# HengyiWang/spann3r

Hardware: NVIDIA H100
Metric: frames/sec (512x384, 10-frame seq) enc->mem-attn->dec->DPT (higher is better)
Workload: dtype bf16x3 (split-bf16 operands, fp32 accumulate; tf32 attention)

## Files before the change

include/spann3r_b200.h:

```cpp
#ifndef SPANN3R_B200_H_
#define SPANN3R_B200_H_

#include <stddef.h>
#include <stdint.h>

#ifdef __cplusplus
extern "C" {
#endif

#define S3R_VERSION 100

enum { S3R_EPI_PLAIN = 0, S3R_EPI_PIXSHUF = 1, S3R_EPI_QKV = 2, S3R_EPI_HEADTAIL = 3 };
enum { S3R_ACT_NONE = 0, S3R_ACT_GELU = 1, S3R_ACT_RELU = 2 };

int s3r_version(void);
int s3r_abi_sizeof(int which );
const char* s3r_last_error(void);
int s3r_device_ok(void);


int s3r_split(const float* x, int64_t ldx, void* hi, void* lo, int64_t ldp, int col0, int64_t rows, int c, int relu,
              void* stream);

int s3r_layernorm(const float* x, int64_t ldx, const float* w, const float* b, int64_t wb_group_stride,
// ... 15 lines not shown
                   void* stream);
int s3r_col2im_3x3s2(const float* cols, int nb, int h, int w, int c, int ho, int wo, float* out, void* stream);

typedef struct s3r_gemm_desc {
  const void* a_hi; const void* a_lo;
  const void* b_hi; const void* b_lo;
  int groups, nb, h, w, kc, taps, n;
  int epi, act, plane_relu, force_bn;
  const float* bias;
  const float* res1; int64_t ldr1;
  const float* res2; int64_t ldr2;
  float* out_f32; int64_t ldo;
  void* out_hi; void* out_lo; int64_t ldp; int plane_col0;
  int ps_s, ps_cout;
  int q_c, q_role_base, q_ntok, q_ntok_pad, q_rope, q_nb;
  const int32_t* q_pos; const float* q_cs;
  float* q_out; float* k_out; float* vt_out; float q_scale;
  const float* ht_w; const float* ht_b; float* ht_pts; float* ht_conf;
  const float* ln_stats; int ln_np; float ln_eps; const float* ln_cs; int a_swap;
  float* stats_out;
  uint64_t* trace;
  int swap_col0; float* k2_out; float* vt2_out;
  int precision;
} s3r_gemm_desc;
int s3r_gemm(const s3r_gemm_desc* d, void* stream);
int s3r_gemm_tile_n(const s3r_gemm_desc* d);
int s3r_gemm_plan_bn(int64_t m_tiles, int n, int sms, int col_align, int force_bn);

int s3r_attention(const float* q, const float* k, const float* vt, int bh, int heads, int nq, int nk, int nk_pad,
                  void* o_hi, void* o_lo, float* o_f32, int64_t ldo, void* stream);

int s3r_conf_score(const float* conf, int64_t n, float* scratch256, float* out, void* stream);
int s3r_conf_score_batched(const float* conf, int batch, int64_t hw, float* scratch, float* out, void* stream);

int s3r_resample_h_u8(const uint8_t* src, int64_t row_stride, int rows, int out_cols, const int32_t* bounds,
                      const int32_t* kk, int ksize, int max_span, uint8_t* dst, void* stream);
int s3r_resample_v_u8_norm(const uint8_t* tmp, int cols, int out_rows, const int32_t* bounds, const int32_t* kk, int ksize,
                           float* dst, void* stream);

int s3r_focal_weiszfeld(const float* pts3d, int b, int h, int w, float ppx, float ppy, int iters, float lo, float hi,
                        float* scratch, float* focal, void* stream);

int s3r_focal_median(const float* pts3d, int b, int h, int w, float ppx, float ppy, float lo, float hi, int32_t* scratch,
                     float* focal, void* stream);

size_t s3r_pnp_workspace_bytes(int b, int n_samples);
int s3r_pnp_ransac(const float* pts3d, const float* img_pts, int b, int64_t n, int width, double fx, double fy, double cx,
                   double cy, float reproj_err, int n_samples, int refine_iters, uint64_t seed, void* workspace,
                   double* out, uint8_t* inlier_mask, void* stream);

// ... 177 lines not shown
```

spann3r_b200/_lib.py:

```python
from __future__ import annotations

import ctypes as C
import os

import torch

_HERE = os.path.dirname(os.path.abspath(__file__))
LIB_PATH = os.environ.get("S3R_LIB", os.path.join(_HERE, "libspann3r_b200.so"))

EPI_PLAIN, EPI_PIXSHUF, EPI_QKV, EPI_HEADTAIL = 0, 1, 2, 3
PRECISION_SPLIT, PRECISION_BF16 = 0, 1
ACT_NONE, ACT_GELU, ACT_RELU = 0, 1, 2

_vp, _i, _i64, _f = C.c_void_p, C.c_int, C.c_int64, C.c_float


class GemmDesc(C.Structure):
    _fields_ = [
        ("a_hi", _vp), ("a_lo", _vp), ("b_hi", _vp), ("b_lo", _vp),
        ("groups", _i), ("nb", _i), ("h", _i), ("w", _i), ("kc", _i), ("taps", _i), ("n", _i),
        ("epi", _i), ("act", _i), ("plane_relu", _i), ("force_bn", _i),
        ("bias", _vp),
        ("res1", _vp), ("ldr1", _i64),
        ("res2", _vp), ("ldr2", _i64),
        ("out_f32", _vp), ("ldo", _i64),
        ("out_hi", _vp), ("out_lo", _vp), ("ldp", _i64), ("plane_col0", _i),
        ("ps_s", _i), ("ps_cout", _i),
        ("q_c", _i), ("q_role_base", _i), ("q_ntok", _i), ("q_ntok_pad", _i), ("q_rope", _i), ("q_nb", _i),
        ("q_pos", _vp), ("q_cs", _vp),
        ("q_out", _vp), ("k_out", _vp), ("vt_out", _vp), ("q_scale", _f),
        ("ht_w", _vp), ("ht_b", _vp), ("ht_pts", _vp), ("ht_conf", _vp),
        ("ln_stats", _vp), ("ln_np", _i), ("ln_eps", _f), ("ln_cs", _vp), ("a_swap", _i),
        ("stats_out", _vp),
        ("trace", _vp),
        ("swap_col0", _i), ("k2_out", _vp), ("vt2_out", _vp),
        ("precision", _i),
    ]


class LossDesc(C.Structure):
    _fields_ = [
        ("frames", _i), ("batch", _i), ("height", _i), ("width", _i),
        ("norm_mode", _i), ("gt_scale", _i), ("fix_first", _i), ("shift_inv", _i), ("scale_inv", _i), ("conf_loss", _i),
        ("has_dist_clip", _i), ("alpha", _f), ("dist_clip", _f),
        ("pose0", _vp), ("gt_pts", C.POINTER(_vp)), ("valid", C.POINTER(_vp)), ("pred", C.POINTER(_vp)),
        ("conf", C.POINTER(_vp)),
    ]


LOSS_RES_HEADER, LOSS_RES_PER_B = 20, 6


class AttnTrainDesc(C.Structure):
    _fields_ = [
        ("batch", _i), ("heads", _i), ("nq", _i), ("nk", _i), ("dh", _i), ("scale", _f),
        ("q", _vp), ("k", _vp), ("v", _vp),
        ("q_stride", _i64 * 3), ("k_stride", _i64 * 3), ("v_stride", _i64 * 3),
    ]

_PROTOS = {
    "s3r_version": (_i, []),
    "s3r_abi_sizeof": (_i, [_i]),
    "s3r_last_error": (C.c_char_p, []),
    "s3r_device_ok": (_i, []),
    "s3r_split": (_i, [_vp, _i64, _vp, _vp, _i64, _i, _i64, _i, _i, _vp]),
    "s3r_layernorm": (_i, [_vp, _i64, _vp, _vp, _i64, _i64, _f, _i64, _i, _vp, _i64, _vp, _vp, _i64, _i, _i64, _vp]),
    "s3r_rope2d_inplace": (_i, [_vp, _vp, _i64, _i, _i, _i64, _i64, _f, _f, _vp]),
    "s3r_im2col_patch16": (_i, [_vp, _i64, _i64, _i64, _i64, _i, _i, _i, _vp, _vp, _vp]),
    "s3r_im2col_3x3s2": (_i, [_vp, _vp, _i, _i, _i, _i, _i, _i, _vp, _vp, _vp]),
    "s3r_upsample2x": (_i, [_vp, _i, _i, _i, _i, _vp, _vp, _vp, _vp]),
    "s3r_conv_wgrad_workspace_bytes": (C.c_size_t, [_i, _i, _i, _i, _i, _i]),
    "s3r_conv_wgrad": (_i, [_vp, _vp, _i64, _vp, _vp, _i64, _i, _i, _i, _i, _i, _i, _vp, C.c_size_t, _vp, _vp]),
    "s3r_col2im_3x3s2": (_i, [_vp, _i, _i, _i, _i, _i, _i, _vp, _vp]),
    "s3r_gemm": (_i, [C.POINTER(GemmDesc), _vp]),
    "s3r_gemm_tile_n": (_i, [C.POINTER(GemmDesc)]),
    "s3r_gemm_plan_bn": (_i, [_i64, _i, _i, _i, _i]),
    "s3r_attention": (_i, [_vp, _vp, _vp, _i, _i, _i, _i, _i, _vp, _vp, _vp, _i64, _vp]),
    "s3r_conf_score": (_i, [_vp, _i64, _vp, _vp, _vp]),
    "s3r_conf_score_batched": (_i, [_vp, _i, _i64, _vp, _vp, _vp]),
    "s3r_dropout_mask": (_i, [_vp, _i64, C.c_uint64, _f, _vp]),
    "s3r_set_option": (_i, [C.c_char_p, _i]),
    "s3r_focal_weiszfeld": (_i, [_vp, _i, _i, _i, _f, _f, _i, _f, _f, _vp, _vp, _vp]),
    "s3r_focal_median": (_i, [_vp, _i, _i, _i, _f, _f, _f, _f, _vp, _vp, _vp]),
    "s3r_pnp_workspace_bytes": (C.c_size_t, [_i, _i]),
    "s3r_pnp_ransac": (_i, [_vp, _vp, _i, _i64, _i, C.c_double, C.c_double, C.c_double, C.c_double, _f, _i, _i, C.c_uint64,
                            _vp, _vp, _vp, _vp]),
    "s3r_pcl_index_bytes": (C.c_size_t, [_i64]),
    "s3r_pcl_index_build": (_i, [_vp, _i, _i64, _vp, _vp, _vp]),
    "s3r_pcl_nearest": (_i, [_vp, _i64, _vp, _i, _i64, _vp, C.c_double, _vp, _vp, _vp]),
    "s3r_pcl_normals": (_i, [_vp, _i64, _i, _vp, _vp]),
    "s3r_pcl_icp_workspace_bytes": (C.c_size_t, []),
    "s3r_pcl_icp": (_i, [_vp, _i, _i64, _vp, _i64, C.c_double, _vp, _i, C.c_double, C.c_double, _vp, _vp, _vp]),
    "s3r_pcl_stats_workspace_bytes": (C.c_size_t, []),
    "s3r_pcl_stats": (_i, [_vp, _i64, C.c_double, _vp, _vp, _vp]),
    "s3r_pcl_abs_dot": (_i, [_vp, _vp, _vp, _i64, _vp, _vp]),
    "s3r_render_workspace_bytes": (C.c_size_t, [_i, _i]),
    "s3r_render_clear": (_i, [_vp, _i, _i, _vp]),
    "s3r_render_splat": (_i, [_vp, _vp, _i64, _i64, _vp, C.c_double, _i, _i, _vp, _vp]),
    "s3r_render_resolve": (_i, [_vp, _vp, _i, _i, _vp, _vp]),
# ... 225 lines not shown
```

spann3r_b200/csrc/capi.cu:

```cuda
#include "../../include/spann3r_b200.h"

#include <cstring>

#include "gemm.cuh"
#include "kernels.cuh"

using namespace s3r;

static inline cudaStream_t S(void* s) { return reinterpret_cast<cudaStream_t>(s); }
static inline __nv_bfloat16* B(void* p) { return reinterpret_cast<__nv_bfloat16*>(p); }
static inline const __nv_bfloat16* B(const void* p) { return reinterpret_cast<const __nv_bfloat16*>(p); }

extern "C" {

int s3r_version(void) { return S3R_VERSION; }
int s3r_abi_sizeof(int which) {
  switch (which) {
    case 0: return (int)sizeof(s3r_gemm_desc);
    case 1: return (int)sizeof(s3r_model_w);
    case 2: return (int)sizeof(s3r_bank);
    case 3: return (int)sizeof(s3r_loss_desc);
    case 4: return (int)sizeof(s3r_attn_train_desc);
  }
  return -1;
// ... 129 lines not shown
    }
    if (d->ln_np < 2 || d->ln_np > 32 || d->ln_np % 2 != 0) {
      set_error("s3r_gemm: folded LayerNorm needs an even ln_np in [2, 32] (kc %% 64 == 0, kc <= 1024), got ln_np=%d",
                d->ln_np);
      return -1;
    }
  }
  if (d->swap_col0 % 256 != 0) {
    set_error("s3r_gemm: swap_col0 must be a multiple of 256");
    return -1;
  }
  if (d->stats_out && d->epi != S3R_EPI_PLAIN) {
    set_error("s3r_gemm: stats_out needs EPI_PLAIN");
    return -1;
  }
  return 0;
}

static int fill_plan(const s3r_gemm_desc* d, GemmPlan* plan) {
  int r = check_desc(d);
  if (r) return r;
  const int force_bn = d->epi == S3R_EPI_HEADTAIL ? (d->force_bn == 128 ? 128 : 1128) : d->force_bn;
  r = gemm_plan_init(plan, B(d->a_hi), B(d->a_lo), B(d->b_hi), B(d->b_lo), d->groups, d->nb, d->h, d->w, d->kc,
                     d->taps, d->n, force_bn, 0, 0, 0, d->precision, d->a_swap ? d->swap_col0 : 0);
  if (r) return r;
  GemmArgs& a = plan->args;
  a.epi = d->epi; a.act = d->act; a.plane_relu = d->plane_relu;
  a.bias = d->bias;
  a.res1 = d->res1; a.ldr1 = (int)d->ldr1;
  a.res2 = d->res2; a.ldr2 = (int)d->ldr2;
  a.out_f32 = d->out_f32; a.ldo = (int)d->ldo;
  a.out_hi = B(d->out_hi); a.out_lo = B(d->out_lo); a.ldp = (int)d->ldp; a.plane_col0 = d->plane_col0;
  if (d->epi == S3R_EPI_PIXSHUF) {
    a.ps_s = d->ps_s; a.ps_cout = d->ps_cout;
    a.out_group_rows = (long long)d->nb * d->h * d->ps_s * d->w * d->ps_s;
  }
  if (d->epi == S3R_EPI_QKV) {
    a.q_C = d->q_c; a.q_role_base = d->q_role_base; a.q_ntok = d->q_ntok; a.q_ntok_pad = d->q_ntok_pad;
    a.q_rope = d->q_rope; a.q_nb = d->q_nb; a.q_pos = d->q_pos;
    a.q_cs = reinterpret_cast<const float2*>(d->q_cs);
    a.q_out = d->q_out; a.k_out = d->k_out; a.vt_out = d->vt_out; a.q_scale = d->q_scale;
    a.k2_out = d->k2_out; a.vt2_out = d->vt2_out;
  }
  if (d->epi == S3R_EPI_HEADTAIL) {
    a.ht_w = d->ht_w; a.ht_b = d->ht_b; a.ht_pts = d->ht_pts; a.ht_conf = d->ht_conf;
  }
  if (d->ln_stats) {
    a.ln_stats = reinterpret_cast<const float2*>(d->ln_stats); a.ln_np = d->ln_np; a.ln_eps = d->ln_eps; a.ln_cs = d->ln_cs;
  }
  a.a_swap = d->a_swap ? 1 : 0;
  a.swap_col0 = d->swap_col0;
  a.stats_out = reinterpret_cast<float2*>(d->stats_out);
  a.trace = reinterpret_cast<unsigned long long*>(d->trace);
  return 0;
}

int s3r_gemm(const s3r_gemm_desc* d, void* stream) {
  GemmPlan plan;
  int r = fill_plan(d, &plan);
  if (r) return r;
  return gemm_launch(plan, S(stream));
}

int s3r_gemm_tile_n(const s3r_gemm_desc* d) {
  GemmPlan plan;
  int r = fill_plan(d, &plan);
  if (r) return r;
  return plan.bn;
}

int s3r_gemm_plan_bn(int64_t m_tiles, int n, int sms, int col_align, int force_bn) {
  if (m_tiles < 1 || n < 1 || sms < 1 || col_align < 0) {
    set_error("s3r_gemm_plan_bn: m_tiles=%lld n=%d sms=%d col_align=%d (positive; col_align >= 0)", (long long)m_tiles,
              n, sms, col_align);
    return -1;
  }
  return gemm_choose_bn(m_tiles, n, sms, col_align, force_bn);
}

int s3r_resample_h_u8(const uint8_t* src, int64_t row_stride, int rows, int out_cols, const int32_t* bounds,
                      const int32_t* kk, int ksize, int max_span, uint8_t* dst, void* stream) {
  return launch_resample_h_u8(src, row_stride, rows, out_cols, bounds, kk, ksize, max_span, dst, S(stream));
}
int s3r_resample_v_u8_norm(const uint8_t* tmp, int cols, int out_rows, const int32_t* bounds, const int32_t* kk, int ksize,
                           float* dst, void* stream) {
  return launch_resample_v_u8_norm(tmp, cols, out_rows, bounds, kk, ksize, dst, S(stream));
}

int s3r_focal_weiszfeld(const float* pts3d, int b, int h, int w, float ppx, float ppy, int iters, float lo, float hi,
                        float* scratch, float* focal, void* stream) {
  return launch_focal_weiszfeld(pts3d, b, h, w, ppx, ppy, iters, lo, hi, scratch, focal, S(stream));
}

// ... 62 lines not shown
  return launch_loss_backward(d, workspace, workspace_bytes, upstream, grad_pred, grad_conf, S(stream));
}

size_t s3r_attn_train_workspace_bytes(const s3r_attn_train_desc* d) { return attn_train_workspace_bytes(d); }
int s3r_attn_train_forward(const s3r_attn_train_desc* d, float* o, float* lse, void* stream) {
  return launch_attn_train_forward(d, o, lse, S(stream));
}
int s3r_attn_train_backward(const s3r_attn_train_desc* d, const float* o, const float* lse, const float* d_o,
                            void* workspace, size_t workspace_bytes, float* dq, float* dk, float* dv, void* stream) {
  return launch_attn_train_backward(d, o, lse, d_o, workspace, workspace_bytes, dq, dk, dv, S(stream));
}

int s3r_conf_score(const float* conf, int64_t n, float* scratch256, float* out, void* stream) {
  return launch_conf_score(conf, n, scratch256, out, S(stream));
}
int s3r_conf_score_batched(const float* conf, int batch, int64_t hw, float* scratch, float* out, void* stream) {
  return launch_conf_score_batched(conf, batch, hw, scratch, out, S(stream));
}

int s3r_set_option(const char* name, int value) {
  s3r::Options& o = s3r::options();
  if (!name) { set_error("s3r_set_option: null name"); return -1; }
  if (!strcmp(name, "prefetch_b")) o.prefetch_b = value;
  else { set_error("s3r_set_option: unknown option '%s' (prefetch_b)", name); return -1; }
  return 0;
}

int s3r_dropout_mask(float* out, int64_t n, uint64_t seed, float p, void* stream) {
  if (!out && n > 0) {
    set_error("s3r_dropout_mask: null output");
    return -1;
  }
  return launch_dropout_mask(out, n, seed, p, S(stream));
}

int s3r_attention(const float* q, const float* k, const float* vt, int bh, int heads, int nq, int nk, int nk_pad,
                  void* o_hi, void* o_lo, float* o_f32, int64_t ldo, void* stream) {
  return launch_attention(q, k, vt, bh, heads, nq, nk, nk_pad, B(o_hi), B(o_lo), o_f32, ldo, S(stream));
}

}
```

spann3r_b200/csrc/common.cuh:

```cuda
#pragma once
#include <cuda.h>
#include <cuda_bf16.h>
#include <cuda_runtime.h>
#include <stdint.h>

#include <cstdlib>
#include <utility>

namespace s3r {

__device__ __forceinline__ uint32_t smem_u32(const void* p) {
  return static_cast<uint32_t>(__cvta_generic_to_shared(p));
}
__device__ __forceinline__ uint32_t lane_id() { return threadIdx.x & 31; }
__device__ __forceinline__ bool elect_one() {
  uint32_t pred = 0;
  asm volatile(
      "{\n\t.reg .pred P1;\n\t"
      "elect.sync _|P1, 0xffffffff;\n\t"
      "selp.u32 %0, 1, 0, P1;\n\t}\n"
      : "=r"(pred));
  return pred != 0;
}

// ... 84 lines not shown
      "l"(reinterpret_cast<uint64_t>(m)), "r"(smem_u32(bar)), "r"(c0), "r"(c1), "r"(c2), "r"(c3)
      : "memory");
}

__device__ __forceinline__ void mbar_arrive_expect_tx_u(uint32_t bar, uint32_t bytes) {
  asm volatile("mbarrier.arrive.expect_tx.shared::cta.b64 _, [%0], %1;" ::"r"(bar), "r"(bytes) : "memory");
}
__device__ __forceinline__ void tma_load_3d_u(uint32_t smem, const CUtensorMap* m, uint32_t bar, int c0, int c1, int c2) {
  asm volatile(
      "cp.async.bulk.tensor.3d.shared::cta.global.mbarrier::complete_tx::bytes [%0], [%1, {%3, %4, %5}], [%2];" ::
          "r"(smem),
      "l"(reinterpret_cast<uint64_t>(m)), "r"(bar), "r"(c0), "r"(c1), "r"(c2)
      : "memory");
}
__device__ __forceinline__ void tma_load_4d_u(uint32_t smem, const CUtensorMap* m, uint32_t bar, int c0, int c1, int c2,
                                              int c3) {
  asm volatile(
      "cp.async.bulk.tensor.4d.shared::cta.global.mbarrier::complete_tx::bytes [%0], [%1, {%3, %4, %5, %6}], "
      "[%2];" ::"r"(smem),
      "l"(reinterpret_cast<uint64_t>(m)), "r"(bar), "r"(c0), "r"(c1), "r"(c2), "r"(c3)
      : "memory");
}

__device__ __forceinline__ uint64_t wgmma_desc_sw128_kmajor(uint32_t smem_addr) {
  uint64_t d = 0;
  d |= (uint64_t)((smem_addr & 0x3FFFF) >> 4);
  d |= (uint64_t)1 << 16;
  d |= (uint64_t)64 << 32;
  d |= (uint64_t)1 << 62;
  return d;
}

__device__ __forceinline__ uint64_t wgmma_desc_sw64_kmajor(uint32_t smem_addr) {
  uint64_t d = 0;
  d |= (uint64_t)((smem_addr & 0x3FFFF) >> 4);
  d |= (uint64_t)1 << 16;
  d |= (uint64_t)32 << 32;
  d |= (uint64_t)2 << 62;
  return d;
}

__device__ __forceinline__ void pdl_launch_dependents() { asm volatile("griddepcontrol.launch_dependents;" ::: "memory"); }
__device__ __forceinline__ void pdl_wait() { asm volatile("griddepcontrol.wait;" ::: "memory"); }

__device__ __forceinline__ unsigned long long globaltimer_ns() {
  unsigned long long t;
  asm volatile("mov.u64 %0, %%globaltimer;" : "=l"(t));
  return t;
}

__device__ __forceinline__ void st_f4(float* p, float a, float b, float c, float d) {
  *reinterpret_cast<float4*>(p) = make_float4(a, b, c, d);
}

struct PerDeviceOnce {
  bool done[64] = {};
  bool& cur() {
    int d = 0;
    cudaGetDevice(&d);
    return done[d & 63];
  }
};

template <typename... KArgs, typename... Args>
inline cudaError_t launch_pdl(void (*kernel)(KArgs...), dim3 grid, dim3 block, size_t smem, cudaStream_t st, Args&&... args) {
  cudaLaunchConfig_t cfg = {};
  cfg.gridDim = grid;
  cfg.blockDim = block;
  cfg.dynamicSmemBytes = smem;
  cfg.stream = st;
  static const bool use_pdl = (getenv("S3R_NO_PDL") == nullptr);
  cudaLaunchAttribute attr[1];
  attr[0].id = cudaLaunchAttributeProgrammaticStreamSerialization;
  attr[0].val.programmaticStreamSerializationAllowed = 1;
  cfg.attrs = attr;
  cfg.numAttrs = use_pdl ? 1 : 0;
  return cudaLaunchKernelEx(&cfg, kernel, std::forward<Args>(args)...);
}

}
```

spann3r_b200/csrc/gemm.cu:

```cuda
#include "gemm.cuh"

#include <cmath>
#include <cstdarg>
#include <cstdio>
#include <cstring>

#include "common.cuh"
#include "gemm_epilogue.cuh"
#include "wgmma.cuh"

namespace s3r {

static constexpr int BM = 128;
static constexpr int BK = 32;
static constexpr CUtensorMapSwizzle kSwizzle = CU_TENSOR_MAP_SWIZZLE_64B;
static constexpr int kEpiWarps = 8;
static constexpr int kNumThreads = 128 + 32 * kEpiWarps;
static constexpr int kSmemMax = 227 * 1024;
static constexpr int kAccLD = 36;
static constexpr int kAccBytes = 2 * BM * kAccLD * 4;

template <int BN, int NP>
struct GemmCfg {
  static constexpr int PLANES = NP == 3 ? 2 : 1;
// ... 22 lines not shown

template <int BN, int EPI, int NP>
__global__ void __launch_bounds__(kNumThreads, 1) gemm_bf16x3_kernel(const __grid_constant__ GemmArgs args) {
  using Cfg = GemmCfg<BN, NP>;
  extern __shared__ uint8_t smem_raw[];
  uint8_t* smem = smem_raw + ((1024u - (smem_u32(smem_raw) & 1023u)) & 1023u);
  uint64_t* bars = reinterpret_cast<uint64_t*>(smem + Cfg::STAGES * Cfg::STAGE);
  uint64_t* full_bar = bars;
  uint64_t* empty_bar = bars + Cfg::STAGES;
  float* sacc = reinterpret_cast<float*>(smem + Cfg::STAGES * Cfg::STAGE + 256);
  float* colv = reinterpret_cast<float*>(reinterpret_cast<uint8_t*>(sacc) + kAccBytes);
  float4* hts = reinterpret_cast<float4*>(reinterpret_cast<uint8_t*>(colv) + Cfg::COLV);

  const int warp = threadIdx.x >> 5;
  const int lane = threadIdx.x & 31;
  const bool trace = blockIdx.x == 0 && args.trace != nullptr;
  if (trace && threadIdx.x == 0) args.trace[0] = globaltimer_ns();

  const int n_tiles = (args.N + BN - 1) / BN;
  const int m_tiles = args.tiles_w * args.tiles_h * args.NB;
  const int tiles_per_group = n_tiles * m_tiles;
  const int total_tiles = tiles_per_group * args.groups;
  const int num_kb = args.taps * args.kpt;

  if (warp == 0 && lane == 0) {
    tma_prefetch_desc(&args.tmA_hi);
    tma_prefetch_desc(&args.tmB_hi);
    if constexpr (NP == 3) {
      tma_prefetch_desc(&args.tmA_lo);
      tma_prefetch_desc(&args.tmB_lo);
    }
    for (int i = 0; i < Cfg::STAGES; ++i) {
      mbar_init(&full_bar[i], 1);
      mbar_init(&empty_bar[i], kEpiWarps);
    }
    fence_barrier_init();
  }
  __syncthreads();
  pdl_launch_dependents();
  if (trace && threadIdx.x == 0) args.trace[1] = globaltimer_ns();
  int pre_b = 0;
  if (warp == 0 && args.b_static && (int)blockIdx.x < total_tiles) {
    const int tile = blockIdx.x;
    const int g = tile / tiles_per_group;
    const int nt = (tile - g * tiles_per_group) % n_tiles;
    const int brow = g * args.b_group_rows + nt * BN;
    pre_b = num_kb < Cfg::STAGES ? num_kb : Cfg::STAGES;
    if (lane == 0) {
      for (int kb = 0; kb < pre_b; ++kb) {
        const int tap = kb / args.kpt, kc = (kb - tap * args.kpt) * BK;
        uint8_t* s = smem + kb * Cfg::STAGE;
        mbar_arrive_expect_tx(&full_bar[kb], Cfg::STAGE);
        tma_load_3d(s + Cfg::B_OFF, &args.tmB_hi, &full_bar[kb], kc, tap, brow);
        if constexpr (NP == 3) tma_load_3d(s + Cfg::B_OFF + Cfg::B_TILE, &args.tmB_lo, &full_bar[kb], kc, tap, brow);
      }
    }
    __syncwarp();
  }
  pdl_wait();
  if (trace && threadIdx.x == 0) args.trace[2] = globaltimer_ns();

  if (warp < 4) {
    asm volatile("setmaxnreg.dec.sync.aligned.u32 40;");
    if (warp == 0) {
      const uint32_t smem_u = __shfl_sync(0xffffffffu, smem_u32(smem), 0);
      const uint32_t full_u = __shfl_sync(0xffffffffu, smem_u32(full_bar), 0);
      int stage = 0;
      uint32_t phase = 0;
      for (int tile = blockIdx.x; tile < total_tiles; tile += gridDim.x) {
        const int g = tile / tiles_per_group;
        const int rem = tile - g * tiles_per_group;
        const int mt = rem / n_tiles;
        const int nt = rem - mt * n_tiles;
        const int tw = mt % args.tiles_w;
        const int th = (mt / args.tiles_w) % args.tiles_h;
        const int nb = mt / (args.tiles_w * args.tiles_h);
        const int w0 = tw * args.bw, h0 = th * args.bh;
        const int img = ((args.a_swap && nt * BN >= args.swap_col0) ? (args.groups - 1 - g) : g) * args.NB + nb;
        const int brow = g * args.b_group_rows + nt * BN;
        int tap = 0, kc = 0, dx = (args.taps == 9) ? -1 : 0, dy = dx;
        for (int kb = 0; kb < num_kb; ++kb) {
          mbar_wait(&empty_bar[stage], phase ^ 1);
          const bool b_done = (tile == (int)blockIdx.x) && (kb < pre_b);
          if (elect_one()) {
            const uint32_t s = smem_u + stage * Cfg::STAGE;
            const uint32_t fb = full_u + stage * 8;
            if (!b_done) mbar_arrive_expect_tx_u(fb, Cfg::STAGE);
            tma_load_4d_u(s, &args.tmA_hi, fb, kc, w0 + dx, h0 + dy, img);
            if constexpr (NP == 3) tma_load_4d_u(s + Cfg::A_TILE, &args.tmA_lo, fb, kc, w0 + dx, h0 + dy, img);
            if (!b_done) {
              tma_load_3d_u(s + Cfg::B_OFF, &args.tmB_hi, fb, kc, tap, brow);
              if constexpr (NP == 3) tma_load_3d_u(s + Cfg::B_OFF + Cfg::B_TILE, &args.tmB_lo, fb, kc, tap, brow);
            }
          }
          __syncwarp();
          kc += BK;
          if (kc >= args.kpt * BK) {
            kc = 0;
            ++tap;
            if (++dx > 1) {
              dx = -1;
              ++dy;
            }
          }
          if (++stage == Cfg::STAGES) {
            stage = 0;
            phase ^= 1;
          }
        }
      }
    }
  } else {
    asm volatile("setmaxnreg.inc.sync.aligned.u32 232;");
    const int cw = warp - 4;
    const int wg = cw >> 2;
    const int wq = cw & 3;
    const int quad = cw & 3;
    const int half = cw >> 2;
    constexpr int NCH = BN / 32;
    constexpr int CH = (NCH + 1) / 2;
    const uint32_t smem_u = __shfl_sync(0xffffffffu, smem_u32(smem), 0);
    int stage = 0;
    uint32_t phase = 0;
    int it = 0;
    for (int tile = blockIdx.x; tile < total_tiles; tile += gridDim.x, ++it) {
      const int g = tile / tiles_per_group;
      const int rem = tile - g * tiles_per_group;
      const int mt = rem / n_tiles;
      const int nt = rem - mt * n_tiles;
      const int tw = mt % args.tiles_w;
      const int th = (mt / args.tiles_w) % args.tiles_h;
      const int nb = mt / (args.tiles_w * args.tiles_h);

      float* sb = colv + (it & 1) * 2 * BN;
      float* scs = sb + BN;
      epi_stage_cols<EPI, BN>(args, sb, scs, g, nt, (int)threadIdx.x - 128, 32 * kEpiWarps);
      const TileGeom tg = make_geom(args, g, nb, th, tw, nt * BN);
      EpiRow er;
      EpiTRows tr;
      epi_tile_pre<EPI, 32>(args, tg, quad, lane, er, tr);
      float4 res[8];
      const int cfirst = nt * BN + half * CH * 32;
      if (cfirst < args.N) epi_prefetch_res<EPI, 32>(args, tr, res, cfirst, lane);
      asm volatile("bar.sync 1, %0;" ::"n"(32 * kEpiWarps) : "memory");
// ... 8 lines not shown
        const uint32_t sa = smem_u + stage * Cfg::STAGE;
        const uint64_t da_hi = wgmma_desc_sw64_kmajor(sa + wg * (64 * BK * 2));
        const uint64_t db_hi = wgmma_desc_sw64_kmajor(sa + Cfg::B_OFF);
        wgmma_fence();
        if constexpr (NP == 3) {
          const uint64_t da_lo = wgmma_desc_sw64_kmajor(sa + Cfg::A_TILE + wg * (64 * BK * 2));
          const uint64_t db_lo = wgmma_desc_sw64_kmajor(sa + Cfg::B_OFF + Cfg::B_TILE);
#pragma unroll
          for (int kk = 0; kk < BK / 16; ++kk) {
            const uint64_t ko = (uint64_t)(kk * 32 >> 4);
            wgmma_bf16<BN>(acc, da_hi + ko, db_lo + ko, 1);
            wgmma_bf16<BN>(acc, da_lo + ko, db_hi + ko, 1);
            wgmma_bf16<BN>(acc, da_hi + ko, db_hi + ko, 1);
          }
        } else {
#pragma unroll
          for (int kk = 0; kk < BK / 16; ++kk) {
            const uint64_t ko = (uint64_t)(kk * 32 >> 4);
            wgmma_bf16<BN>(acc, da_hi + ko, db_hi + ko, 1);
          }
        }
        wgmma_commit();
        wgmma_wait<1>();
        if (prev >= 0) {
          __syncwarp();
          if (lane == 0) mbar_arrive(&empty_bar[prev]);
        }
        prev = stage;
        if (++stage == Cfg::STAGES) {
          stage = 0;
          phase ^= 1;
        }
      }
      wgmma_wait<0>();
      if (prev >= 0) {
        __syncwarp();
        if (lane == 0) mbar_arrive(&empty_bar[prev]);
      }
      if (trace && it == 0 && threadIdx.x == 128) args.trace[4] = globaltimer_ns();

      float ht_acc[4] = {0.f, 0.f, 0.f, 0.f};
#pragma unroll
      for (int cc = 0; cc < CH; ++cc) {
        if (cc > 0) asm volatile("bar.sync 1, %0;" ::"n"(32 * kEpiWarps) : "memory");
#pragma unroll
        for (int h = 0; h < 2; ++h) {
          if (h * CH + cc >= NCH) continue;
          float* dst = sacc + h * (BM * kAccLD);
#pragma unroll
          for (int ii = 0; ii < 4; ++ii) {
            const int i = (h * CH + cc) * 4 + ii;
            const int r = wg * 64 + wq * 16 + (lane >> 2);
            const int c = ii * 8 + 2 * (lane & 3);
            *reinterpret_cast<float2*>(dst + r * kAccLD + c) = make_float2(acc[4 * i], acc[4 * i + 1]);
            *reinterpret_cast<float2*>(dst + (r + 8) * kAccLD + c) = make_float2(acc[4 * i + 2], acc[4 * i + 3]);
          }
        }
        asm volatile("bar.sync 1, %0;" ::"n"(32 * kEpiWarps) : "memory");
        float* myrows = sacc + half * (BM * kAccLD) + quad * 32 * kAccLD;
        float v[32];
        {
// ... 6 lines not shown
        }
        __syncwarp();
        const int c = half * CH + cc;
        const int col0 = nt * BN + c * 32;
        if (col0 < args.N && (NCH % 2 == 0 || c < NCH)) {
          const int res_next = (cc + 1 < CH && (NCH % 2 == 0 || c + 1 < NCH) && col0 + 32 < args.N) ? col0 + 32 : -1;
          epi_chunk<EPI, 32>(args, v, sb + c * 32, scs + c * 32, myrows, tg, er, tr, res, col0, res_next, lane, ht_acc);
        }
      }

      if constexpr (EPI == EPI_HEADTAIL) {
        float4* slot = hts + (quad * 2 + (it & 1)) * 32;
        if (half == 1) slot[lane] = make_float4(ht_acc[0], ht_acc[1], ht_acc[2], ht_acc[3]);
        asm volatile("bar.sync %0, 64;" ::"r"(2 + quad) : "memory");
        if (half == 0) {
          const float4 p = slot[lane];
          ht_acc[0] += p.x; ht_acc[1] += p.y; ht_acc[2] += p.z; ht_acc[3] += p.w;
          epi_headtail_finish(args, tg, er, ht_acc);
        }
      }
    }
    if (trace && threadIdx.x == 128) args.trace[5] = globaltimer_ns();
  }
  if (trace && threadIdx.x == 128) args.trace[6] = globaltimer_ns();
}

static thread_local char g_err[512] = "";
const char* last_error() { return g_err; }
void set_error(const char* fmt, ...) {
  va_list ap;
  va_start(ap, fmt);
  vsnprintf(g_err, sizeof(g_err), fmt, ap);
  va_end(ap);
}

typedef CUresult (*PFN_encodeTiled)(CUtensorMap*, CUtensorMapDataType, cuuint32_t, void*, const cuuint64_t*,
                                    const cuuint64_t*, const cuuint32_t*, const cuuint32_t*, CUtensorMapInterleave,
                                    CUtensorMapSwizzle, CUtensorMapL2promotion, CUtensorMapFloatOOBfill);
static PFN_encodeTiled get_encode() {
  static PFN_encodeTiled fn = nullptr;
  if (!fn) {
    void* p = nullptr;
    cudaDriverEntryPointQueryResult qres;
    if (cudaGetDriverEntryPoint("cuTensorMapEncodeTiled", &p, cudaEnableDefault, &qres) != cudaSuccess ||
        qres != cudaDriverEntryPointSuccess)
      return nullptr;
// ... 69 lines not shown
      return -1;
    }
    const int bn = fb > 128 ? 128 : fb;
    if (!fits(bn)) {
      set_error("gemm_plan_init: force_bn %d: a %d-wide tile would straddle swap_col0 = %d", force_bn, bn, col_align);
      return -1;
    }
    return bn;
  }
  if (col_align % 64 != 0) {
    set_error("gemm_plan_init: swap_col0 = %d is not a multiple of 64 (no tile width fits it)", col_align);
    return -1;
  }
  int bn = 64;
  double best = cost(64, 24.0);
  if (fits(96) && cost(96, 28.0) <= best) {
    bn = 96;
    best = cost(96, 28.0);
  }
  if (N > 64 && fits(128) && cost(128, 32.0) <= best) bn = 128;
  return bn;
}

int gemm_plan_init(GemmPlan* plan, const __nv_bfloat16* a_hi, const __nv_bfloat16* a_lo,
                   const __nv_bfloat16* b_hi, const __nv_bfloat16* b_lo, int groups, int NB, int H, int W, int Kc,
                   int taps, int N, int force_bn, long long lda, long long ldb, long long b_group_rows, int precision,
                   int col_align) {
  memset(plan, 0, sizeof(*plan));
  if (precision != GEMM_SPLIT && precision != GEMM_BF16) {
    set_error("gemm_plan_init: precision %d (0 = split bf16, 1 = one bf16 product)", precision);
    return -1;
  }
  plan->precision = precision;
  GemmArgs& a = plan->args;
  if (lda == 0) lda = Kc;
  if (ldb == 0) ldb = (long long)Kc * taps;
  if (b_group_rows == 0) b_group_rows = N;
  if (lda % 8 != 0 || ldb % 8 != 0 || (taps != 1 && taps != 9) || (taps == 9 && Kc % 8 != 0)) {
    set_error("gemm_plan_init: unsupported shape Kc=%d N=%d taps=%d lda=%lld ldb=%lld (row strides must be multiples "
              "of 8 elements, taps in {1,9})", Kc, N, taps, lda, ldb);
    return -1;
  }
  a.b_group_rows = (int)b_group_rows;
  a.W = W; a.H = H; a.NB = NB; a.N = N; a.Kc = Kc; a.taps = taps;
  a.kpt = (Kc + BK - 1) / BK;
  a.bw = W >= 128 ? 128 : next_pow2(W);
  a.bh = 128 / a.bw;
  a.tiles_w = (W + a.bw - 1) / a.bw;
  a.tiles_h = (H + a.bh - 1) / a.bh;
  a.out_group_rows = (long long)NB * H * W;
  const long long m_tiles = (long long)a.tiles_w * a.tiles_h * NB * groups;
  const int bn = gemm_choose_bn(m_tiles, N, num_sms(), col_align, force_bn);
  if (bn < 0) return -1;
  plan->bn = bn;

  const uint64_t esz = 2;
  {
    uint64_t dims[4] = {(uint64_t)Kc, (uint64_t)W, (uint64_t)H, (uint64_t)NB * groups};
    uint64_t str[3] = {(uint64_t)lda * esz, (uint64_t)lda * W * esz, (uint64_t)lda * W * H * esz};
    uint32_t box[4] = {(uint32_t)BK, (uint32_t)a.bw, (uint32_t)a.bh, 1};
    int r;
    if ((r = encode_tmap(&a.tmA_hi, CU_TENSOR_MAP_DATA_TYPE_BFLOAT16, 4, a_hi, dims, str, box, kSwizzle))) return r;
    if (precision == GEMM_SPLIT &&
        (r = encode_tmap(&a.tmA_lo, CU_TENSOR_MAP_DATA_TYPE_BFLOAT16, 4, a_lo, dims, str, box, kSwizzle)))
      return r;
  }
  {
    uint64_t dims[3] = {(uint64_t)Kc, (uint64_t)taps, (uint64_t)(b_group_rows * (groups - 1) + N)};
    uint64_t str[2] = {(uint64_t)(taps == 1 ? ldb : Kc) * esz, (uint64_t)ldb * esz};
    uint32_t box[3] = {(uint32_t)BK, 1, (uint32_t)bn};
    int r;
    if ((r = encode_tmap(&a.tmB_hi, CU_TENSOR_MAP_DATA_TYPE_BFLOAT16, 3, b_hi, dims, str, box, kSwizzle))) return r;
    if (precision == GEMM_SPLIT &&
        (r = encode_tmap(&a.tmB_lo, CU_TENSOR_MAP_DATA_TYPE_BFLOAT16, 3, b_lo, dims, str, box, kSwizzle)))
      return r;
  }
  const long long n_tiles = (N + bn - 1) / bn;
  const long long total = m_tiles * n_tiles;
  a.groups = groups;
  plan->grid = dim3((unsigned)((total < num_sms()) ? total : num_sms()), 1, 1);
  plan->flops = 2.0 * (double)NB * H * W * groups * (double)N * (double)Kc * taps;
  return 0;
}

template <int BN, int EPI, int NP>
static int launch_bn(const GemmPlan& plan, cudaStream_t stream) {
  using Cfg = GemmCfg<BN, NP>;
  static PerDeviceOnce once;
  bool& attr_set = once.cur();
  if (!attr_set) {
    cudaError_t e =
        cudaFuncSetAttribute(gemm_bf16x3_kernel<BN, EPI, NP>, cudaFuncAttributeMaxDynamicSharedMemorySize, Cfg::SMEM);
    if (e != cudaSuccess) {
      set_error("cudaFuncSetAttribute(smem=%d): %s", Cfg::SMEM, cudaGetErrorString(e));
      return -5;
    }
    attr_set = true;
  }
  cudaError_t e = launch_pdl(gemm_bf16x3_kernel<BN, EPI, NP>, plan.grid, dim3(kNumThreads), Cfg::SMEM, stream, plan.args);
  if (e != cudaSuccess) {
    set_error("gemm launch failed: %s", cudaGetErrorString(e));
    return -6;
  }
  return 0;
}

template <int BN, int NP>
static int launch_epi(const GemmPlan& plan, cudaStream_t stream) {
  switch (plan.args.epi) {
    case EPI_PLAIN: return launch_bn<BN, EPI_PLAIN, NP>(plan, stream);
    case EPI_PIXSHUF: return launch_bn<BN, EPI_PIXSHUF, NP>(plan, stream);
    case EPI_QKV: return launch_bn<BN, EPI_QKV, NP>(plan, stream);
    case EPI_HEADTAIL:
      if constexpr (NP == 3 && BN != 96) return launch_bn<BN, EPI_HEADTAIL, NP>(plan, stream);
      break;
  }
  set_error("gemm_launch: bad epilogue mode %d", plan.args.epi);
  return -1;
}

template <int NP>
static int launch_np(const GemmPlan& plan, cudaStream_t stream) {
// ... 20 lines not shown
```

spann3r_b200/csrc/gemm.cuh:

```cuda
#pragma once
#include <cuda.h>
#include <cuda_bf16.h>
#include <cuda_runtime.h>
#include <stdint.h>

namespace s3r {

enum EpiMode : int {
  EPI_PLAIN = 0,
  EPI_PIXSHUF = 1,
  EPI_QKV = 2,
  EPI_HEADTAIL = 3,
};
enum Act : int { ACT_NONE = 0, ACT_GELU = 1, ACT_RELU = 2 };
enum GemmPrecision : int { GEMM_SPLIT = 0, GEMM_BF16 = 1 };

struct GemmArgs {
  alignas(64) CUtensorMap tmA_hi;
  alignas(64) CUtensorMap tmA_lo;
  alignas(64) CUtensorMap tmB_hi;
  alignas(64) CUtensorMap tmB_lo;
  int groups;
  int W, H, NB;
  int bw, bh;
  int tiles_w, tiles_h;
  int N;
  int Kc, taps, kpt;
  int b_group_rows;
  int epi, act, plane_relu;
  const float* bias;
  const float* res1; int ldr1;
  const float* res2; int ldr2;
  float* out_f32; int ldo;
  __nv_bfloat16* out_hi; __nv_bfloat16* out_lo; int ldp; int plane_col0;
  long long out_group_rows;
  const float2* ln_stats; int ln_np; float ln_eps;
  const float* ln_cs;
  int b_static;
  int a_swap;
  int swap_col0;
  float2* stats_out;
  unsigned long long* trace;
  int ps_s, ps_cout;
  int q_C, q_role_base, q_ntok, q_ntok_pad, q_rope, q_nb;
  const int* q_pos;
  const float2* q_cs;
  float* q_out; float* k_out; float* vt_out;
  float* k2_out; float* vt2_out;
  float q_scale;
  const float* ht_w;
  const float* ht_b;
  float* ht_pts;
  float* ht_conf;
};

struct GemmPlan {
  GemmArgs args;
  dim3 grid;
  int bn;
  int precision;
  int b_static;
  double flops;
};

int gemm_plan_init(GemmPlan* plan,
                   const __nv_bfloat16* a_hi, const __nv_bfloat16* a_lo,
                   const __nv_bfloat16* b_hi, const __nv_bfloat16* b_lo,
                   int groups, int NB, int H, int W, int Kc, int taps, int N, int force_bn = 0,
                   long long lda = 0, long long ldb = 0, long long b_group_rows = 0, int precision = GEMM_SPLIT,
                   int col_align = 0);
int gemm_choose_bn(long long m_tiles, int N, int sms, int col_align, int force_bn);
int gemm_launch(const GemmPlan& plan, cudaStream_t stream);

struct Options {
  int prefetch_b = 1;
};
Options& options();
int num_sms();

int encode_tmap(CUtensorMap* out, CUtensorMapDataType dt, int rank, const void* base, const uint64_t* dims,
                const uint64_t* strides_bytes, const uint32_t* box,
                CUtensorMapSwizzle swizzle = CU_TENSOR_MAP_SWIZZLE_128B);
const char* last_error();
void set_error(const char* fmt, ...);

}
```

Baseline: 92.68.

## Share split-bf16 operand loads across 2-CTA clusters via TMA multicast

Adds an optional 2-CTA cluster mode to the split-bf16 GEMM. When paired CTAs work on tiles that use the same A or B operand, each CTA loads either the hi or lo plane and multicasts it to both, which halves per-CTA global and L2 traffic for that operand. Empty barriers now count arrivals from both CTAs through remote mbarrier arrives, and a heuristic chooses the share mode from tile counts, K depth and cluster occupancy. The cost is cluster synchronisation, coupled pipeline progress between the paired CTAs, and possibly fewer resident CTAs.

```diff
diff --git a/include/spann3r_b200.h b/include/spann3r_b200.h
--- a/include/spann3r_b200.h
+++ b/include/spann3r_b200.h
@@ -61,10 +61,14 @@
   uint64_t* trace;
   int swap_col0; float* k2_out; float* vt2_out;
   int precision;
+  int force_share;
 } s3r_gemm_desc;
 int s3r_gemm(const s3r_gemm_desc* d, void* stream);
 int s3r_gemm_tile_n(const s3r_gemm_desc* d);
+int s3r_gemm_share(const s3r_gemm_desc* d);
 int s3r_gemm_plan_bn(int64_t m_tiles, int n, int sms, int col_align, int force_bn);
+int s3r_gemm_plan_share(int64_t m_tiles, int groups, int n_tiles, int bn, int precision, int col_align, int num_kb,
+                        int sms, int cluster_slots, int force_share);
 
 int s3r_attention(const float* q, const float* k, const float* vt, int bh, int heads, int nq, int nk, int nk_pad,
                   void* o_hi, void* o_lo, float* o_f32, int64_t ldo, void* stream);
diff --git a/spann3r_b200/_lib.py b/spann3r_b200/_lib.py
--- a/spann3r_b200/_lib.py
+++ b/spann3r_b200/_lib.py
@@ -34,7 +34,7 @@
         ("stats_out", _vp),
         ("trace", _vp),
         ("swap_col0", _i), ("k2_out", _vp), ("vt2_out", _vp),
-        ("precision", _i),
+        ("precision", _i), ("force_share", _i),
     ]
 
 
@@ -75,6 +75,8 @@
     "s3r_gemm": (_i, [C.POINTER(GemmDesc), _vp]),
     "s3r_gemm_tile_n": (_i, [C.POINTER(GemmDesc)]),
     "s3r_gemm_plan_bn": (_i, [_i64, _i, _i, _i, _i]),
+    "s3r_gemm_share": (_i, [C.POINTER(GemmDesc)]),
+    "s3r_gemm_plan_share": (_i, [_i64, _i, _i, _i, _i, _i, _i, _i, _i, _i]),
     "s3r_attention": (_i, [_vp, _vp, _vp, _i, _i, _i, _i, _i, _vp, _vp, _vp, _i64, _vp]),
     "s3r_conf_score": (_i, [_vp, _i64, _vp, _vp, _vp]),
     "s3r_conf_score_batched": (_i, [_vp, _i, _i64, _vp, _vp, _vp]),
diff --git a/spann3r_b200/csrc/capi.cu b/spann3r_b200/csrc/capi.cu
--- a/spann3r_b200/csrc/capi.cu
+++ b/spann3r_b200/csrc/capi.cu
@@ -175,7 +175,7 @@
   if (r) return r;
   const int force_bn = d->epi == S3R_EPI_HEADTAIL ? (d->force_bn == 128 ? 128 : 1128) : d->force_bn;
   r = gemm_plan_init(plan, B(d->a_hi), B(d->a_lo), B(d->b_hi), B(d->b_lo), d->groups, d->nb, d->h, d->w, d->kc,
-                     d->taps, d->n, force_bn, 0, 0, 0, d->precision, d->a_swap ? d->swap_col0 : 0);
+                     d->taps, d->n, force_bn, 0, 0, 0, d->precision, d->a_swap ? d->swap_col0 : 0, d->force_share);
   if (r) return r;
   GemmArgs& a = plan->args;
   a.epi = d->epi; a.act = d->act; a.plane_relu = d->plane_relu;
@@ -222,6 +222,24 @@
   return plan.bn;
 }
 
+int s3r_gemm_share(const s3r_gemm_desc* d) {
+  GemmPlan plan;
+  int r = fill_plan(d, &plan);
+  if (r) return r;
+  return plan.args.share;
+}
+
+int s3r_gemm_plan_share(int64_t m_tiles, int groups, int n_tiles, int bn, int precision, int col_align, int num_kb,
+                        int sms, int cluster_slots, int force_share) {
+  if (m_tiles < 1 || groups < 1 || n_tiles < 1 || (bn != 64 && bn != 96 && bn != 128) || col_align < 0 || num_kb < 1 ||
+      sms < 1 || cluster_slots < 0) {
+    set_error("s3r_gemm_plan_share: m_tiles=%lld groups=%d n_tiles=%d bn=%d col_align=%d num_kb=%d sms=%d "
+              "cluster_slots=%d", (long long)m_tiles, groups, n_tiles, bn, col_align, num_kb, sms, cluster_slots);
+    return -1;
+  }
+  return gemm_choose_share(m_tiles, groups, n_tiles, bn, precision, col_align, num_kb, sms, cluster_slots, force_share);
+}
+
 int s3r_gemm_plan_bn(int64_t m_tiles, int n, int sms, int col_align, int force_bn) {
   if (m_tiles < 1 || n < 1 || sms < 1 || col_align < 0) {
     set_error("s3r_gemm_plan_bn: m_tiles=%lld n=%d sms=%d col_align=%d (positive; col_align >= 0)", (long long)m_tiles,
@@ -330,7 +348,8 @@
   s3r::Options& o = s3r::options();
   if (!name) { set_error("s3r_set_option: null name"); return -1; }
   if (!strcmp(name, "prefetch_b")) o.prefetch_b = value;
-  else { set_error("s3r_set_option: unknown option '%s' (prefetch_b)", name); return -1; }
+  else if (!strcmp(name, "multicast")) o.multicast = value;
+  else { set_error("s3r_set_option: unknown option '%s' (prefetch_b, multicast)", name); return -1; }
   return 0;
 }
 
diff --git a/spann3r_b200/csrc/common.cuh b/spann3r_b200/csrc/common.cuh
--- a/spann3r_b200/csrc/common.cuh
+++ b/spann3r_b200/csrc/common.cuh
@@ -130,6 +130,38 @@
       : "memory");
 }
 
+__device__ __forceinline__ uint32_t cluster_ctarank() {
+  uint32_t r;
+  asm volatile("mov.u32 %0, %%cluster_ctarank;" : "=r"(r));
+  return r;
+}
+__device__ __forceinline__ void cluster_sync() {
+  asm volatile("barrier.cluster.arrive.release.aligned;\n\tbarrier.cluster.wait.acquire.aligned;" ::: "memory");
+}
+__device__ __forceinline__ void mbar_arrive_remote(uint32_t bar, uint32_t cta) {
+  asm volatile(
+      "{\n\t.reg .b32 rb;\n\t"
+      "mapa.shared::cluster.u32 rb, %0, %1;\n\t"
+      "mbarrier.arrive.shared::cluster.b64 _, [rb];\n\t}" ::"r"(bar), "r"(cta)
+      : "memory");
+}
+__device__ __forceinline__ void tma_load_3d_mc(uint32_t smem, const CUtensorMap* m, uint32_t bar, int c0, int c1, int c2,
+                                               uint16_t mask) {
+  asm volatile(
+      "cp.async.bulk.tensor.3d.shared::cluster.global.mbarrier::complete_tx::bytes.multicast::cluster"
+      " [%0], [%1, {%3, %4, %5}], [%2], %6;" ::"r"(smem),
+      "l"(reinterpret_cast<uint64_t>(m)), "r"(bar), "r"(c0), "r"(c1), "r"(c2), "h"(mask)
+      : "memory");
+}
+__device__ __forceinline__ void tma_load_4d_mc(uint32_t smem, const CUtensorMap* m, uint32_t bar, int c0, int c1, int c2,
+                                               int c3, uint16_t mask) {
+  asm volatile(
+      "cp.async.bulk.tensor.4d.shared::cluster.global.mbarrier::complete_tx::bytes.multicast::cluster"
+      " [%0], [%1, {%3, %4, %5, %6}], [%2], %7;" ::"r"(smem),
+      "l"(reinterpret_cast<uint64_t>(m)), "r"(bar), "r"(c0), "r"(c1), "r"(c2), "r"(c3), "h"(mask)
+      : "memory");
+}
+
 __device__ __forceinline__ uint64_t wgmma_desc_sw128_kmajor(uint32_t smem_addr) {
   uint64_t d = 0;
   d |= (uint64_t)((smem_addr & 0x3FFFF) >> 4);
@@ -171,19 +203,33 @@
 };
 
 template <typename... KArgs, typename... Args>
-inline cudaError_t launch_pdl(void (*kernel)(KArgs...), dim3 grid, dim3 block, size_t smem, cudaStream_t st, Args&&... args) {
+inline cudaError_t launch_pdl_cluster(void (*kernel)(KArgs...), dim3 grid, dim3 block, size_t smem, cudaStream_t st,
+                                      int cluster, Args&&... args) {
   cudaLaunchConfig_t cfg = {};
   cfg.gridDim = grid;
   cfg.blockDim = block;
   cfg.dynamicSmemBytes = smem;
   cfg.stream = st;
   static const bool use_pdl = (getenv("S3R_NO_PDL") == nullptr);
-  cudaLaunchAttribute attr[1];
-  attr[0].id = cudaLaunchAttributeProgrammaticStreamSerialization;
-  attr[0].val.programmaticStreamSerializationAllowed = 1;
+  cudaLaunchAttribute attr[2];
+  int n = 0;
+  if (use_pdl) {
+    attr[n].id = cudaLaunchAttributeProgrammaticStreamSerialization;
+    attr[n++].val.programmaticStreamSerializationAllowed = 1;
+  }
+  if (cluster > 1) {
+    attr[n].id = cudaLaunchAttributeClusterDimension;
+    attr[n].val.clusterDim.x = (unsigned)cluster;
+    attr[n].val.clusterDim.y = 1;
+    attr[n++].val.clusterDim.z = 1;
+  }
   cfg.attrs = attr;
-  cfg.numAttrs = use_pdl ? 1 : 0;
+  cfg.numAttrs = n;
   return cudaLaunchKernelEx(&cfg, kernel, std::forward<Args>(args)...);
 }
-
-}
+template <typename... KArgs, typename... Args>
+inline cudaError_t launch_pdl(void (*kernel)(KArgs...), dim3 grid, dim3 block, size_t smem, cudaStream_t st, Args&&... args) {
+  return launch_pdl_cluster(kernel, grid, block, smem, st, 1, std::forward<Args>(args)...);
+}
+
+}
diff --git a/spann3r_b200/csrc/gemm.cu b/spann3r_b200/csrc/gemm.cu
--- a/spann3r_b200/csrc/gemm.cu
+++ b/spann3r_b200/csrc/gemm.cu
@@ -68,6 +68,8 @@
   const int tiles_per_group = n_tiles * m_tiles;
   const int total_tiles = tiles_per_group * args.groups;
   const int num_kb = args.taps * args.kpt;
+  const int share = NP == 3 ? args.share : SHARE_NONE;
+  const uint32_t rank = share ? cluster_ctarank() : 0;
 
   if (warp == 0 && lane == 0) {
     tma_prefetch_desc(&args.tmA_hi);
@@ -78,11 +80,12 @@
     }
     for (int i = 0; i < Cfg::STAGES; ++i) {
       mbar_init(&full_bar[i], 1);
-      mbar_init(&empty_bar[i], kEpiWarps);
+      mbar_init(&empty_bar[i], share ? 2 * kEpiWarps : kEpiWarps);
     }
     fence_barrier_init();
   }
-  __syncthreads();
+  if (share) cluster_sync();
+  else __syncthreads();
   pdl_launch_dependents();
   if (trace && threadIdx.x == 0) args.trace[1] = globaltimer_ns();
   int pre_b = 0;
@@ -97,8 +100,13 @@
         const int tap = kb / args.kpt, kc = (kb - tap * args.kpt) * BK;
         uint8_t* s = smem + kb * Cfg::STAGE;
         mbar_arrive_expect_tx(&full_bar[kb], Cfg::STAGE);
-        tma_load_3d(s + Cfg::B_OFF, &args.tmB_hi, &full_bar[kb], kc, tap, brow);
-        if constexpr (NP == 3) tma_load_3d(s + Cfg::B_OFF + Cfg::B_TILE, &args.tmB_lo, &full_bar[kb], kc, tap, brow);
+        if (share == SHARE_B) {
+          tma_load_3d_mc(smem_u32(s + Cfg::B_OFF + rank * Cfg::B_TILE), rank ? &args.tmB_lo : &args.tmB_hi,
+                         smem_u32(&full_bar[kb]), kc, tap, brow, 0x3);
+        } else {
+          tma_load_3d(s + Cfg::B_OFF, &args.tmB_hi, &full_bar[kb], kc, tap, brow);
+          if constexpr (NP == 3) tma_load_3d(s + Cfg::B_OFF + Cfg::B_TILE, &args.tmB_lo, &full_bar[kb], kc, tap, brow);
+        }
       }
     }
     __syncwarp();
@@ -132,11 +140,21 @@
             const uint32_t s = smem_u + stage * Cfg::STAGE;
             const uint32_t fb = full_u + stage * 8;
             if (!b_done) mbar_arrive_expect_tx_u(fb, Cfg::STAGE);
-            tma_load_4d_u(s, &args.tmA_hi, fb, kc, w0 + dx, h0 + dy, img);
-            if constexpr (NP == 3) tma_load_4d_u(s + Cfg::A_TILE, &args.tmA_lo, fb, kc, w0 + dx, h0 + dy, img);
+            if (share == SHARE_A) {
+              tma_load_4d_mc(s + rank * Cfg::A_TILE, rank ? &args.tmA_lo : &args.tmA_hi, fb, kc, w0 + dx, h0 + dy, img,
+                             0x3);
+            } else {
+              tma_load_4d_u(s, &args.tmA_hi, fb, kc, w0 + dx, h0 + dy, img);
+              if constexpr (NP == 3) tma_load_4d_u(s + Cfg::A_TILE, &args.tmA_lo, fb, kc, w0 + dx, h0 + dy, img);
+            }
             if (!b_done) {
-              tma_load_3d_u(s + Cfg::B_OFF, &args.tmB_hi, fb, kc, tap, brow);
-              if constexpr (NP == 3) tma_load_3d_u(s + Cfg::B_OFF + Cfg::B_TILE, &args.tmB_lo, fb, kc, tap, brow);
+              if (share == SHARE_B) {
+                tma_load_3d_mc(s + Cfg::B_OFF + rank * Cfg::B_TILE, rank ? &args.tmB_lo : &args.tmB_hi, fb, kc, tap,
+                               brow, 0x3);
+              } else {
+                tma_load_3d_u(s + Cfg::B_OFF, &args.tmB_hi, fb, kc, tap, brow);
+                if constexpr (NP == 3) tma_load_3d_u(s + Cfg::B_OFF + Cfg::B_TILE, &args.tmB_lo, fb, kc, tap, brow);
+              }
             }
           }
           __syncwarp();
@@ -166,6 +184,14 @@
     constexpr int NCH = BN / 32;
     constexpr int CH = (NCH + 1) / 2;
     const uint32_t smem_u = __shfl_sync(0xffffffffu, smem_u32(smem), 0);
+    const uint32_t empty_u = __shfl_sync(0xffffffffu, smem_u32(empty_bar), 0);
+    auto release = [&](int s) {
+      __syncwarp();
+      if (lane == 0) {
+        mbar_arrive(&empty_bar[s]);
+        if (share) mbar_arrive_remote(empty_u + s * 8, rank ^ 1);
+      }
+    };
     int stage = 0;
     uint32_t phase = 0;
     int it = 0;
@@ -220,10 +246,7 @@
         }
         wgmma_commit();
         wgmma_wait<1>();
-        if (prev >= 0) {
-          __syncwarp();
-          if (lane == 0) mbar_arrive(&empty_bar[prev]);
-        }
+        if (prev >= 0) release(prev);
         prev = stage;
         if (++stage == Cfg::STAGES) {
           stage = 0;
@@ -231,10 +254,7 @@
         }
       }
       wgmma_wait<0>();
-      if (prev >= 0) {
-        __syncwarp();
-        if (lane == 0) mbar_arrive(&empty_bar[prev]);
-      }
+      if (prev >= 0) release(prev);
       if (trace && it == 0 && threadIdx.x == 128) args.trace[4] = globaltimer_ns();
 
       float ht_acc[4] = {0.f, 0.f, 0.f, 0.f};
@@ -287,6 +307,7 @@
     }
     if (trace && threadIdx.x == 128) args.trace[5] = globaltimer_ns();
   }
+  if (share) cluster_sync();
   if (trace && threadIdx.x == 128) args.trace[6] = globaltimer_ns();
 }
 
@@ -402,10 +423,100 @@
   return bn;
 }
 
+static constexpr int kPairMinKb = 64;
+int gemm_choose_share(long long m_tiles, int groups, int n_tiles, int bn, int precision, int col_align, int num_kb,
+                      int sms, int cluster_slots, int force_share) {
+  const long long total = m_tiles * n_tiles;
+  const bool split = precision == GEMM_SPLIT;
+  const bool can_a = split && n_tiles % 2 == 0 && col_align % (2 * bn) == 0;
+  const bool can_b = split && n_tiles == 1 && groups > 0 && m_tiles % groups == 0 && (m_tiles / groups) % 2 == 0;
+  switch (force_share) {
+    case FORCE_SHARE_OFF: return SHARE_NONE;
+    case FORCE_SHARE_A:
+    case FORCE_SHARE_B: {
+      const bool a = force_share == FORCE_SHARE_A;
+      if (!(a ? can_a : can_b)) {
+        set_error("gemm_plan_init: force_share %d: share mode %s needs split precision and %s (n_tiles %d at bn %d, "
+                  "%lld row tiles in %d groups, swap_col0 %d)", force_share, a ? "A" : "B",
+                  a ? "an even number of column tiles, swap_col0 a multiple of 2 bn" : "one column tile, even row tiles per group",
+                  n_tiles, bn, m_tiles, groups, col_align);
+        return -1;
+      }
+      if (cluster_slots < 2) {
+        set_error("gemm_plan_init: force_share %d: no 2-CTA cluster of this kernel fits the device", force_share);
+        return -1;
+      }
+      return a ? SHARE_A : SHARE_B;
+    }
+    case FORCE_SHARE_AUTO: break;
+    default:
+      set_error("gemm_plan_init: force_share %d (0 auto, 1 A, 2 B, 3 off)", force_share);
+      return -1;
+  }
+  if ((!can_a && !can_b) || cluster_slots < 2 || sms < 1) return SHARE_NONE;
+  if (total <= sms && num_kb < kPairMinKb) return SHARE_NONE;
+  if ((total + cluster_slots - 1) / cluster_slots > (total + sms - 1) / sms) return SHARE_NONE;
+  return can_a ? SHARE_A : SHARE_B;
+}
+
+template <int BN, int EPI, int NP>
+static int set_smem_attr() {
+  static PerDeviceOnce once;
+  bool& attr_set = once.cur();
+  if (!attr_set) {
+    cudaError_t e = cudaFuncSetAttribute(gemm_bf16x3_kernel<BN, EPI, NP>, cudaFuncAttributeMaxDynamicSharedMemorySize,
+                                         GemmCfg<BN, NP>::SMEM);
+    if (e != cudaSuccess) {
+      set_error("cudaFuncSetAttribute(smem=%d): %s", GemmCfg<BN, NP>::SMEM, cudaGetErrorString(e));
+      return -5;
+    }
+    attr_set = true;
+  }
+  return 0;
+}
+
+template <int BN>
+static int cluster_slots_bn() {
+  static int slots[64];
+  static PerDeviceOnce once;
+  int dev = 0;
+  cudaGetDevice(&dev);
+  bool& done = once.cur();
+  if (!done) {
+    int n = 0;
+    if (set_smem_attr<BN, EPI_PLAIN, 3>() == 0) {
+      cudaLaunchConfig_t cfg = {};
+      cfg.gridDim = dim3((unsigned)(num_sms() / 2 * 2));
+      cfg.blockDim = dim3(kNumThreads);
+      cfg.dynamicSmemBytes = GemmCfg<BN, 3>::SMEM;
+      cudaLaunchAttribute attr;
+      attr.id = cudaLaunchAttributeClusterDimension;
+      attr.val.clusterDim.x = 2;
+      attr.val.clusterDim.y = 1;
+      attr.val.clusterDim.z = 1;
+      cfg.attrs = &attr;
+      cfg.numAttrs = 1;
+      if (cudaOccupancyMaxActiveClusters(&n, gemm_bf16x3_kernel<BN, EPI_PLAIN, 3>, &cfg) != cudaSuccess) n = 0;
+    }
+    cudaGetLastError();
+    slots[dev & 63] = 2 * n;
+    done = true;
+  }
+  return slots[dev & 63];
+}
+
+static int cluster_slots(int bn) {
+  switch (bn) {
+    case 64: return cluster_slots_bn<64>();
+    case 96: return cluster_slots_bn<96>();
+    default: return cluster_slots_bn<128>();
+  }
+}
+
 int gemm_plan_init(GemmPlan* plan, const __nv_bfloat16* a_hi, const __nv_bfloat16* a_lo,
                    const __nv_bfloat16* b_hi, const __nv_bfloat16* b_lo, int groups, int NB, int H, int W, int Kc,
                    int taps, int N, int force_bn, long long lda, long long ldb, long long b_group_rows, int precision,
-                   int col_align) {
+                   int col_align, int force_share) {
   memset(plan, 0, sizeof(*plan));
   if (precision != GEMM_SPLIT && precision != GEMM_BF16) {
     set_error("gemm_plan_init: precision %d (0 = split bf16, 1 = one bf16 product)", precision);
@@ -433,6 +544,16 @@
   const int bn = gemm_choose_bn(m_tiles, N, num_sms(), col_align, force_bn);
   if (bn < 0) return -1;
   plan->bn = bn;
+  const int n_tiles = (N + bn - 1) / bn;
+  const int num_kb = taps * ((Kc + BK - 1) / BK);
+  if (force_share == FORCE_SHARE_AUTO && !options().multicast) force_share = FORCE_SHARE_OFF;
+  int share = gemm_choose_share(m_tiles, groups, n_tiles, bn, precision, col_align, num_kb, num_sms(), num_sms(),
+                                force_share);
+  if (share < 0) return -1;
+  const int slots = share != SHARE_NONE ? cluster_slots(bn) : 0;
+  if (share != SHARE_NONE)
+    share = gemm_choose_share(m_tiles, groups, n_tiles, bn, precision, col_align, num_kb, num_sms(), slots, force_share);
+  if (share < 0) return -1;
 
   const uint64_t esz = 2;
   {
@@ -455,10 +576,12 @@
         (r = encode_tmap(&a.tmB_lo, CU_TENSOR_MAP_DATA_TYPE_BFLOAT16, 3, b_lo, dims, str, box, kSwizzle)))
       return r;
   }
-  const long long n_tiles = (N + bn - 1) / bn;
   const long long total = m_tiles * n_tiles;
   a.groups = groups;
-  plan->grid = dim3((unsigned)((total < num_sms()) ? total : num_sms()), 1, 1);
+  a.share = share;
+  plan->cluster = share != SHARE_NONE ? 2 : 1;
+  const int slots_all = share != SHARE_NONE ? slots : num_sms();
+  plan->grid = dim3((unsigned)((total < slots_all) ? total : slots_all), 1, 1);
   plan->flops = 2.0 * (double)NB * H * W * groups * (double)N * (double)Kc * taps;
   return 0;
 }
@@ -466,18 +589,9 @@
 template <int BN, int EPI, int NP>
 static int launch_bn(const GemmPlan& plan, cudaStream_t stream) {
   using Cfg = GemmCfg<BN, NP>;
-  static PerDeviceOnce once;
-  bool& attr_set = once.cur();
-  if (!attr_set) {
-    cudaError_t e =
-        cudaFuncSetAttribute(gemm_bf16x3_kernel<BN, EPI, NP>, cudaFuncAttributeMaxDynamicSharedMemorySize, Cfg::SMEM);
-    if (e != cudaSuccess) {
-      set_error("cudaFuncSetAttribute(smem=%d): %s", Cfg::SMEM, cudaGetErrorString(e));
-      return -5;
-    }
-    attr_set = true;
-  }
-  cudaError_t e = launch_pdl(gemm_bf16x3_kernel<BN, EPI, NP>, plan.grid, dim3(kNumThreads), Cfg::SMEM, stream, plan.args);
+  if (int r = set_smem_attr<BN, EPI, NP>()) return r;
+  cudaError_t e = launch_pdl_cluster(gemm_bf16x3_kernel<BN, EPI, NP>, plan.grid, dim3(kNumThreads), Cfg::SMEM, stream,
+                                     plan.cluster, plan.args);
   if (e != cudaSuccess) {
     set_error("gemm launch failed: %s", cudaGetErrorString(e));
     return -6;
diff --git a/spann3r_b200/csrc/gemm.cuh b/spann3r_b200/csrc/gemm.cuh
--- a/spann3r_b200/csrc/gemm.cuh
+++ b/spann3r_b200/csrc/gemm.cuh
@@ -14,6 +14,8 @@
 };
 enum Act : int { ACT_NONE = 0, ACT_GELU = 1, ACT_RELU = 2 };
 enum GemmPrecision : int { GEMM_SPLIT = 0, GEMM_BF16 = 1 };
+enum GemmShare : int { SHARE_NONE = 0, SHARE_A = 1, SHARE_B = 2 };
+enum GemmForceShare : int { FORCE_SHARE_AUTO = 0, FORCE_SHARE_A = 1, FORCE_SHARE_B = 2, FORCE_SHARE_OFF = 3 };
 
 struct GemmArgs {
   alignas(64) CUtensorMap tmA_hi;
@@ -39,6 +41,7 @@
   int b_static;
   int a_swap;
   int swap_col0;
+  int share;
   float2* stats_out;
   unsigned long long* trace;
   int ps_s, ps_cout;
@@ -57,6 +60,7 @@
 struct GemmPlan {
   GemmArgs args;
   dim3 grid;
+  int cluster;
   int bn;
   int precision;
   int b_static;
@@ -68,12 +72,15 @@
                    const __nv_bfloat16* b_hi, const __nv_bfloat16* b_lo,
                    int groups, int NB, int H, int W, int Kc, int taps, int N, int force_bn = 0,
                    long long lda = 0, long long ldb = 0, long long b_group_rows = 0, int precision = GEMM_SPLIT,
-                   int col_align = 0);
+                   int col_align = 0, int force_share = FORCE_SHARE_AUTO);
 int gemm_choose_bn(long long m_tiles, int N, int sms, int col_align, int force_bn);
+int gemm_choose_share(long long m_tiles, int groups, int n_tiles, int bn, int precision, int col_align, int num_kb,
+                      int sms, int cluster_slots, int force_share);
 int gemm_launch(const GemmPlan& plan, cudaStream_t stream);
 
 struct Options {
   int prefetch_b = 1;
+  int multicast = 1;
 };
 Options& options();
 int num_sms();
```

After: 95.26, median of 6. 2.8% higher.
